# MinghanLi/STMask

Hardware: AMD Instinct MI355X
Metric: frames/sec at 360x640 R50-DCN-FPN (STMask hot path, fp32) (higher is better)
Workload: dtype f32

## Files before the change

### stmask_amd/csrc/head_sparse.hip

```cpp
#include <algorithm>

#include "stm_common.h"

namespace {

enum { CTL_RAW = 0,
       CTL_N = 1,
       CTL_FILL = 2,
       CTL_GATE_A = 3,
       CTL_GATE_B = 4,
       CTL_DENSE = 5,
       CTL_OVERFLOW = 6,
       CTL_GATE_POS = 7,
       CTL_INTS = 8 };

struct Levels {
    int n, B;
    int start[9], h[8], w[8];
};

__device__ __forceinline__ void decode_pixel(const Levels& L, int m, int& l, int& b, int& y, int& x)
{
    l = 0;
#pragma unroll
    for (int i = 1; i < 8; ++i)
        if (i < L.n && m >= L.start[i]) l = i;
    const int r = m - L.start[l], hw = L.h[l] * L.w[l];
    b = r / hw;
    const int p = r - b * hw;
    y = p / L.w[l];
    x = p - y * L.w[l];
}

struct CandArgs {
    const float* cls[4];
    int K, ld, n_cls, n_pixels, capacity;
    float thresh;
    int* list;
    int* ctl;
    int* flags;
    Levels L;
};

__global__ __launch_bounds__(256) void head_clear_kernel(int* ctl, int* flags, int n_pixels)
{
    const int i = blockIdx.x * 256 + threadIdx.x;
    if (i < n_pixels) flags[i] = 0;
    else if (i < n_pixels + CTL_INTS) ctl[i - n_pixels] = 0;
}

__device__ __forceinline__ void list_pixel(const CandArgs& a, int m)
{
    if (atomicCAS(a.flags + m, 0, 1) != 0) return;
    const int i = atomicAdd(a.ctl + CTL_RAW, 1);
    if (i < a.capacity) a.list[i] = m;
}

constexpr int CAND_PX = 64;

__global__ __launch_bounds__(256) void head_candidates_kernel(const CandArgs a, int vec)
{
    extern __shared__ float slab[];
    __shared__ unsigned kept_s[CAND_PX];
    const int stride = a.n_cls | 1;
    const int m0 = blockIdx.x * CAND_PX;
    const int rows = min(CAND_PX, a.n_pixels - m0);
    if (threadIdx.x < CAND_PX) kept_s[threadIdx.x] = 0u;
    for (int k = 0; k < a.K; ++k) {
        const float* src = a.cls[k] + (int64_t)m0 * a.ld;
        float* dst = slab + k * CAND_PX * stride;
        if (vec) {
            const int nv = (a.n_cls + 3) >> 2;
            for (int idx = threadIdx.x; idx < rows * nv; idx += 256) {
                const int r = idx / nv, v = idx - r * nv;
                const float4 q = *reinterpret_cast<const float4*>(src + (int64_t)r * a.ld + 4 * v);
                float* d = dst + r * stride + 4 * v;
                d[0] = q.x;
                if (4 * v + 1 < a.n_cls) d[1] = q.y;
// ... 4 lines not shown
            for (int idx = threadIdx.x; idx < rows * a.n_cls; idx += 256) {
                const int r = idx / a.n_cls, c = idx - r * a.n_cls;
                dst[r * stride + c] = src[(int64_t)r * a.ld + c];
            }
        }
    }
    __syncthreads();
    const int k = threadIdx.x / CAND_PX, r = threadIdx.x - k * CAND_PX;
    if (k < a.K && r < rows) {
        const float* row = slab + (k * CAND_PX + r) * stride;
        float mf = row[1];
        for (int c = 2; c < a.n_cls; ++c) mf = row[c] > mf ? row[c] : mf;
        const float mx = row[0] > mf ? row[0] : mf;
        float sum = 0.0f;
        for (int c = 0; c < a.n_cls; ++c) sum += expf(row[c] - mx);
        const float p = expf(mf - mx) / sum;
        if (p > a.thresh) atomicOr(&kept_s[r], 1u << k);
    }
    __syncthreads();
    if (threadIdx.x >= rows) return;
    const unsigned kept = kept_s[threadIdx.x];
    if (!kept) return;
    const int m = m0 + threadIdx.x;
    list_pixel(a, m);
    int l, b, y, x;
    decode_pixel(a.L, m, l, b, y, x);
    const int hw = a.L.h[l] * a.L.w[l], pix = y * a.L.w[l] + x;
    for (int kk = 0; kk < a.K; ++kk)
        if (kept >> kk & 1) list_pixel(a, a.L.start[l] + b * hw + (pix * a.K + kk) % hw);
}

__global__ void head_control_kernel(int* ctl, int capacity, int n_pixels, int px_a, int px_b)
{
    if (threadIdx.x || blockIdx.x) return;
    const int raw = ctl[CTL_RAW];
    const bool over = raw > capacity;
    const int n = over ? 0 : raw;
    const int fill = min(capacity, (n + 255) & ~255);
    ctl[CTL_N] = n;
    ctl[CTL_FILL] = fill;
    ctl[CTL_GATE_A] = fill * px_a;
    ctl[CTL_GATE_B] = fill * px_b;
    ctl[CTL_DENSE] = over ? n_pixels : 0;
    ctl[CTL_OVERFLOW] = over ? 1 : 0;
    ctl[CTL_GATE_POS] = n;
}

struct GatherArgs {
    const uint8_t* src;
    uint8_t* dst;
    int rows;
    int64_t src_np, dst_np;
    int S;
    const int* list;
    const int* ctl;
    Levels L;
};

__global__ __launch_bounds__(256) void head_patch_gather_kernel(const GatherArgs a)
{
    const int n = a.ctl[CTL_N], fill = a.ctl[CTL_FILL];
    const int SS = a.S * a.S, half = a.S >> 1;
    const int row_groups = (a.rows + 15) >> 4;
    const int64_t units = (int64_t)fill * SS * row_groups;
    const int lane = threadIdx.x & 63;
    const int sub_row = lane >> 2, chunk = lane & 3;
    for (int64_t u = (int64_t)blockIdx.x * 4 + (threadIdx.x >> 6); u < units; u += (int64_t)gridDim.x * 4) {
        const int64_t pp = u / row_groups;
// ... 26 lines not shown
        if (y - half >= 0 && y + half < L.h[l] && x - half >= 0 && x + half < L.w[l]) continue;
        const int work = SS * rows * 4;
        for (int t = threadIdx.x; t < work; t += 256) {
            const int chunk = t & 3, r = (t >> 2) % rows, q = (t >> 2) / rows;
            const int yy = y + q / S - half, xx = x + q % S - half;
            if ((unsigned)yy < (unsigned)L.h[l] && (unsigned)xx < (unsigned)L.w[l]) continue;
            *reinterpret_cast<uint4*>(planes + ((int64_t)r * np + (int64_t)i * SS + q) * 64 + chunk * 16) = make_uint4(0u, 0u, 0u, 0u);
        }
    }
}

struct AsmArgs {
    const float* cls[4];
    const float* small[4];
    const float* trk[4];
    float *conf, *loc, *mask, *track, *cen;
    int B, K, n_levels, n_cls, mask_dim, embed, gpad, cls_ld, small_ld, trk_ld, N;
    int lvl_start[9], lvl_hw[8], lvl_off[8];
    int vec4;
    int row_mul, row_add;
    const int* list;
    const int* ctl;
    int capacity;
};

__device__ __forceinline__ void assemble_rest(const AsmArgs& a, const float* sm, const float* tk, int64_t o, int64_t cen_idx, int sub)
{
    if (sub < 4) a.loc[o * 4 + sub] = sm[1 + sub];
    for (int c = sub; c < a.mask_dim; c += 16) a.mask[o * a.mask_dim + c] = sm[a.gpad + c];
    if (sub == 0) a.cen[cen_idx] = tanhf(sm[0]);
    float ss = 0.0f;
    if (a.vec4) {
        typedef float f4 __attribute__((ext_vector_type(4)));
        f4 v[4];
        const int nv = a.embed >> 2;
#pragma unroll
        for (int q = 0; q < 4; ++q) {
            const int c4 = sub + 16 * q;
            if (c4 < nv) {
                v[q] = *reinterpret_cast<const f4*>(tk + 4 * c4);
                ss = fmaf(v[q].x, v[q].x, ss); ss = fmaf(v[q].y, v[q].y, ss); ss = fmaf(v[q].z, v[q].z, ss); ss = fmaf(v[q].w, v[q].w, ss);
            }
        }
#pragma unroll
        for (int d = 8; d >= 1; d >>= 1) ss += __shfl_xor(ss, d);
        const float inv = 1.0f / fmaxf(sqrtf(ss), 1e-12f);
// ... 19 lines not shown
    const int64_t row = (int64_t)stm_xcd_block(((int64_t)a.B * a.N + 15) >> 4) * 16 + (threadIdx.x >> 4);
    if (row < 0 || row >= (int64_t)a.B * a.N) return;
    const int b = (int)(row / a.N), n = (int)(row - (int64_t)b * a.N);
    int l = 0;
#pragma unroll
    for (int i = 1; i < 8; ++i)
        if (i < a.n_levels && n >= a.lvl_off[i]) l = i;
    const int r = n - a.lvl_off[l];
    const int p = r / a.K, k = r - p * a.K;
    const int hw = a.lvl_hw[l];
    const int64_t src = (int64_t)a.lvl_start[l] + (int64_t)b * hw + p;
    const int64_t o = (int64_t)b * a.N + n;
    if (MODE == 0) {
        const float* cl = a.cls[k] + src * a.cls_ld;
        for (int c = sub; c < a.n_cls; c += 16) a.conf[o * a.n_cls + c] = cl[c];
    } else {
        assemble_rest(a, a.small[k] + src * a.small_ld, a.trk[k] + src * a.trk_ld, o, (int64_t)b * a.N + a.lvl_off[l] + (int64_t)k * hw + p, sub);
    }
}

__global__ __launch_bounds__(256) void head_assemble_listed_kernel(const AsmArgs a)
{
    const int n_pos = a.ctl[CTL_N];
    const int sub = threadIdx.x & 15;
    const int64_t units = (int64_t)n_pos * a.K;
    for (int64_t u = (int64_t)blockIdx.x * 16 + (threadIdx.x >> 4); u < units; u += (int64_t)gridDim.x * 16) {
        const int i = (int)(u / a.K), k = (int)(u - (int64_t)i * a.K);
        const int m = a.list[i];
        int l = 0;
#pragma unroll
        for (int j = 1; j < 8; ++j)
            if (j < a.n_levels && m >= a.lvl_start[j]) l = j;
        const int hw = a.lvl_hw[l];
        const int rr = m - a.lvl_start[l];
        const int b = rr / hw, p = rr - b * hw;
        const int nn = a.lvl_off[l] + p * a.K + k;
        const int64_t o = (int64_t)b * a.N + nn;
        const int64_t src = (int64_t)i * a.row_mul + a.row_add;
        assemble_rest(a, a.small[k] + src * a.small_ld, a.trk[k] + src * a.trk_ld, o, (int64_t)b * a.N + a.lvl_off[l] + (int64_t)k * hw + p, sub);
    }
}

bool fill_levels(Levels& L, int n_levels, int B, const int* lvl_start, const int* lvl_h, const int* lvl_w)
{
    if (n_levels <= 0 || n_levels > 8 || B <= 0 || !lvl_start || !lvl_h || !lvl_w || lvl_start[0] != 0) return false;
    L.n = n_levels; L.B = B;
    for (int l = 0; l < 8; ++l) {
        L.start[l] = l < n_levels ? lvl_start[l] : 0;
        L.h[l] = l < n_levels ? lvl_h[l] : 1;
        L.w[l] = l < n_levels ? lvl_w[l] : 1;
        if (l < n_levels && (lvl_h[l] <= 0 || lvl_w[l] <= 0 || lvl_start[l + 1] - lvl_start[l] != B * lvl_h[l] * lvl_w[l])) return false;
    }
    L.start[8] = 0;
    L.start[n_levels] = lvl_start[n_levels];
    return true;
}

}

extern "C" int stm_head_candidates_f32(const float* const* cls_logits, int K, int ld, int n_cls, float conf_thresh, int capacity,
                                       int patch_pixels_a, int patch_pixels_b, int n_levels, int B, const int* lvl_start, const int* lvl_h,
                                       const int* lvl_w, int* flags, int* list, int* ctl, stm_stream_t stream)
{
    const char* who = "stm_head_candidates_f32";
    STM_REQUIRE(cls_logits && list && ctl && flags, STM_ENULL, "%s: NULL argument", who);
    CandArgs a;
    STM_REQUIRE(fill_levels(a.L, n_levels, B, lvl_start, lvl_h, lvl_w), STM_EINVAL, "%s: bad level table", who);
    const int n_pixels = a.L.start[n_levels];
    STM_REQUIRE(K > 0 && K <= 4 && n_cls >= 2 && ld >= n_cls && n_pixels > 0 && capacity > 0 && patch_pixels_a > 0 && patch_pixels_b > 0 &&
                    (int64_t)capacity * std::max(patch_pixels_a, patch_pixels_b) < ((int64_t)1 << 30), STM_EINVAL, "%s: bad sizes", who);
    for (int k = 0; k < 4; ++k) {
        a.cls[k] = k < K ? cls_logits[k] : nullptr;
        STM_REQUIRE(k >= K || a.cls[k], STM_ENULL, "%s: input %d is NULL", who, k);
    }
    a.K = K; a.ld = ld; a.n_cls = n_cls; a.n_pixels = n_pixels; a.capacity = capacity; a.thresh = conf_thresh; a.list = list; a.ctl = ctl;
    a.flags = flags;
    hipLaunchKernelGGL(head_clear_kernel, dim3(stm_cdiv(n_pixels + CTL_INTS, 256)), dim3(256), 0, stm_hs(stream), ctl, flags, n_pixels);
    STM_CHECK_LAUNCH("head_clear_kernel");
    int vec = ld % 4 == 0 && 4 * ((n_cls + 3) / 4) <= ld;
    for (int k = 0; k < K; ++k) vec = vec && ((uintptr_t)a.cls[k] % 16) == 0;
    const size_t lds = (size_t)K * CAND_PX * (n_cls | 1) * sizeof(float);
    STM_REQUIRE(lds <= 48 * 1024, STM_EUNSUPPORTED, "%s: %d classes x %d shapes do not fit the staging buffer", who, n_cls, K);
    hipLaunchKernelGGL(head_candidates_kernel, dim3(stm_cdiv(n_pixels, CAND_PX)), dim3(256), lds, stm_hs(stream), a, vec);
    STM_CHECK_LAUNCH("head_candidates_kernel");
    hipLaunchKernelGGL(head_control_kernel, dim3(1), dim3(64), 0, stm_hs(stream), ctl, capacity, n_pixels, patch_pixels_a, patch_pixels_b);
    STM_CHECK_LAUNCH("head_control_kernel");
    return STM_OK;
}

extern "C" int stm_head_patch_gather(const void* src_planes, long long src_np, void* dst_planes, int side, int n_planes, int slabs,
                                     int capacity, int n_levels, int B, const int* lvl_start, const int* lvl_h, const int* lvl_w, const int* list,
                                     const int* ctl, stm_stream_t stream)
{
    const char* who = "stm_head_patch_gather";
    STM_REQUIRE(src_planes && dst_planes && list && ctl, STM_ENULL, "%s: NULL argument", who);
    STM_REQUIRE(n_planes > 0 && slabs > 0 && capacity > 0 && side > 0 && (side & 1) && src_np > 0 &&
                    (uintptr_t)src_planes % 16 == 0 && (uintptr_t)dst_planes % 16 == 0, STM_EINVAL, "%s: bad sizes or alignment", who);
    GatherArgs a;
    STM_REQUIRE(fill_levels(a.L, n_levels, B, lvl_start, lvl_h, lvl_w), STM_EINVAL, "%s: bad level table", who);
    STM_REQUIRE(src_np >= a.L.start[n_levels], STM_EINVAL, "%s: the source planes hold fewer pixels than the levels", who);
    a.src = static_cast<const uint8_t*>(src_planes); a.dst = static_cast<uint8_t*>(dst_planes);
    a.rows = n_planes * slabs; a.src_np = src_np; a.dst_np = (int64_t)capacity * side * side; a.S = side;
    a.list = list; a.ctl = ctl;
    const int64_t units = (int64_t)capacity * side * side * ((a.rows + 15) / 16);
    const unsigned grid = (unsigned)std::min<int64_t>((units + 3) / 4, 16384);
    hipLaunchKernelGGL(head_patch_gather_kernel, dim3(grid), dim3(256), 0, stm_hs(stream), a);
    STM_CHECK_LAUNCH("head_patch_gather_kernel");
    return STM_OK;
}
// ... 2 lines not shown
                                   const int* lvl_h, const int* lvl_w, const int* list, const int* ctl, stm_stream_t stream)
{
    const char* who = "stm_head_patch_mask";
    STM_REQUIRE(planes && list && ctl, STM_ENULL, "%s: NULL argument", who);
    STM_REQUIRE(n_planes > 0 && slabs > 0 && capacity > 0 && side > 0 && (side & 1) && (uintptr_t)planes % 16 == 0, STM_EINVAL, "%s: bad sizes or alignment", who);
    Levels L;
    STM_REQUIRE(fill_levels(L, n_levels, B, lvl_start, lvl_h, lvl_w), STM_EINVAL, "%s: bad level table", who);
    hipLaunchKernelGGL(head_patch_mask_kernel, dim3(std::min(capacity, 2048)), dim3(256), 0, stm_hs(stream), static_cast<uint8_t*>(planes), n_planes * slabs,
                       (int64_t)capacity * side * side, side, list, ctl, L);
    STM_CHECK_LAUNCH("head_patch_mask_kernel");
    return STM_OK;
}

extern "C" int stm_head_assemble_sparse_f32(const float* const* cls_logits, int cls_ld, const float* const* small, const float* const* trk,
                                            const float* const* small_dense, const float* const* trk_dense, const stm_head_layout* L,
                                            int row_mul, int row_add, const int* list, const int* ctl, int capacity, float* conf, float* loc,
                                            float* mask, float* track, float* centerness, stm_stream_t stream)
{
    const char* who = "stm_head_assemble_sparse_f32";
    STM_REQUIRE(cls_logits && small && trk && small_dense && trk_dense && L && list && ctl && conf && loc && mask && track && centerness, STM_ENULL,
                "%s: NULL argument", who);
    STM_REQUIRE(L->B > 0 && L->K > 0 && L->K <= 4 && L->n_levels > 0 && L->n_levels <= 8 && L->n_cls > 0 && cls_ld >= L->n_cls && L->mask_dim > 0 &&
                    L->mask_dim <= L->group_pad && L->embed_dim > 0 && L->group_pad >= 5 && L->small_ld >= L->group_pad + L->mask_dim &&
                    L->trk_ld >= L->embed_dim && capacity > 0 && row_mul > 0 && row_add >= 0 && row_add < row_mul, STM_EINVAL, "%s: bad layout", who);
    AsmArgs a;
    a.conf = conf; a.loc = loc; a.mask = mask; a.track = track; a.cen = centerness;
    a.B = L->B; a.K = L->K; a.n_levels = L->n_levels; a.n_cls = L->n_cls; a.mask_dim = L->mask_dim; a.embed = L->embed_dim;
    a.gpad = L->group_pad; a.cls_ld = cls_ld; a.small_ld = L->small_ld; a.trk_ld = L->trk_ld;
    a.row_mul = row_mul; a.row_add = row_add; a.list = list; a.ctl = ctl; a.capacity = capacity;
    int off = 0, start = 0;
    for (int l = 0; l < 8; ++l) {
        a.lvl_start[l] = l < L->n_levels ? L->lvl_start[l] : 0;
        a.lvl_hw[l] = l < L->n_levels ? L->lvl_hw[l] : 1;
        a.lvl_off[l] = off;
        if (l < L->n_levels) {
            STM_REQUIRE(L->lvl_hw[l] > 0 && L->lvl_start[l] == start, STM_EINVAL, "%s: level %d: bad pixel range", who, l);
            off += L->lvl_hw[l] * L->K;
            start += L->B * L->lvl_hw[l];
        }
    }
    a.lvl_start[8] = 0;
    a.N = off;
    const int64_t rows = (int64_t)a.B * a.N;
    const bool al = a.embed % 4 == 0 && a.embed <= 256 && a.trk_ld % 4 == 0 && ((uintptr_t)track % 16) == 0;
    auto set = [&](const float* const* sm, const float* const* tk) -> bool {
        a.vec4 = al;
        for (int k = 0; k < 4; ++k) {
            a.cls[k] = k < a.K ? cls_logits[k] : nullptr;
            a.small[k] = k < a.K ? sm[k] : nullptr;
            a.trk[k] = k < a.K ? tk[k] : nullptr;
            if (k < a.K && !(a.cls[k] && a.small[k] && a.trk[k])) return false;
// ... 15 lines not shown
```

### stmask_amd/ops.py

```python
import ctypes
import os

import torch

from . import _lib
from ._lib import DeformGeom, StmError, c_p, call


def _pair(v):
    return (v, v) if isinstance(v, int) else tuple(v)


def _dev(*ts):
    for t in ts:
        if t is not None and not t.is_cuda:
            raise StmError("stmask_amd ops need tensors on the MI355X (got a CPU tensor); there is no CPU fallback")


def _f32c(t):
    if t.dtype != torch.float32:
        raise StmError(f"expected float32, got {t.dtype}")
    return t if t.is_contiguous() else t.contiguous()


# ... 1579 lines not shown
    return out


def head_assemble(small, trk, B, sizes, n_cls, mask_dim, embed_dim, group_pad):
    _dev(*small, *trk)
    K = len(small)
    L, start = _head_layout(B, K, sizes, n_cls, mask_dim, embed_dim, group_pad, small[0].shape[-1], trk[0].shape[-1])
    N = K * sum(h * w for h, w in sizes)
    for t in list(small) + list(trk):
        if t.dtype != torch.float32 or not t.is_contiguous() or t.shape[0] != start:
            raise StmError("head_assemble: inputs must be contiguous fp32 matrices over all level pixels")
    dev = small[0].device
    conf = torch.empty(B, N, n_cls, device=dev)
    loc = torch.empty(B, N, 4, device=dev)
    mask = torch.empty(B, N, mask_dim, device=dev)
    track = torch.empty(B, N, embed_dim, device=dev)
    cen = torch.empty(B, N, 1, device=dev)
    call("stm_head_assemble_f32", _ptr4(small), _ptr4(trk), ctypes.byref(L), _p(conf), _p(loc), _p(mask), _p(track), _p(cen), _stream())
    return conf, loc, mask, track, cen


HEAD_CTL_RAW, HEAD_CTL_N, HEAD_CTL_FILL, HEAD_CTL_GATE_A, HEAD_CTL_GATE_B, HEAD_CTL_DENSE, HEAD_CTL_OVERFLOW, HEAD_CTL_INTS = 0, 1, 2, 3, 4, 5, 6, 8
HEAD_CTL_GATE_POS = 7


def conv_set_pixel_gate(ctl, index):
    _lib.lib().stm_conv_set_pixel_gate(ctl.data_ptr() + 4 * index)


def _level_arrays(B, sizes):
    n = len(sizes)
    st, hh, ww = (ctypes.c_int * 9)(), (ctypes.c_int * 8)(), (ctypes.c_int * 8)()
    start = 0
    for l, (h, w) in enumerate(sizes):
        st[l], hh[l], ww[l] = start, h, w
        start += B * h * w
    st[n] = start
    return n, st, hh, ww, start


def _head_layout(B, K, sizes, n_cls, mask_dim, embed_dim, group_pad, small_ld, trk_ld):
    L = _lib.HeadLayout()
    L.B, L.K, L.n_levels, L.n_cls, L.mask_dim, L.embed_dim, L.group_pad = B, K, len(sizes), n_cls, mask_dim, embed_dim, group_pad
    L.small_ld, L.trk_ld = small_ld, trk_ld
    start = 0
    for l, (h, w) in enumerate(sizes):
        L.lvl_start[l], L.lvl_hw[l] = start, h * w
        start += B * h * w
    return L, start


def _ptr4(ts):
    return (ctypes.c_void_p * 4)(*([t.data_ptr() for t in ts] + [0] * (4 - len(ts))))


def head_candidates(cls_logits, n_cls, conf_thresh, capacity, patch_pixels_a, patch_pixels_b, B, sizes):
    _dev(*cls_logits)
    n_px, ld = cls_logits[0].shape
    n, st, hh, ww, total = _level_arrays(B, sizes)
    for t in cls_logits:
        if t.dtype != torch.float32 or not t.is_contiguous() or tuple(t.shape) != (n_px, ld) or n_px != total:
            raise StmError("head_candidates: inputs must be contiguous fp32 matrices over all level pixels")
    dev = cls_logits[0].device
    lst = torch.empty(capacity, dtype=torch.int32, device=dev)
    ctl = torch.empty(HEAD_CTL_INTS, dtype=torch.int32, device=dev)
    flags = torch.empty(n_px, dtype=torch.int32, device=dev)
    call("stm_head_candidates_f32", _ptr4(cls_logits), len(cls_logits), ld, n_cls, conf_thresh, capacity, patch_pixels_a, patch_pixels_b, n, B, st,
         hh, ww, _p(flags), _p(lst), _p(ctl), _stream())
    return lst, ctl


def head_patch_gather(src, dst, side, capacity, B, sizes, lst, ctl):
    _dev(src, dst)
    if (src.dim() != 4 or dst.dim() != 4 or src.shape[3] != 32 or src.element_size() != 2 or dst.dtype != src.dtype or not src.is_contiguous()
            or not dst.is_contiguous() or tuple(dst.shape) != (src.shape[0], src.shape[1], capacity * side * side, 32)):
        raise StmError(f"head_patch_gather: planes {tuple(src.shape)} -> {tuple(dst.shape)} do not fit capacity {capacity}, side {side}")
    n, st, hh, ww, _ = _level_arrays(B, sizes)
    call("stm_head_patch_gather", _p(src), src.shape[2], _p(dst), side, src.shape[0], src.shape[1], capacity, n, B, st, hh, ww, _p(lst), _p(ctl),
         _stream())
    return dst


def head_patch_mask(planes, side, capacity, B, sizes, lst, ctl):
    _dev(planes)
    if planes.dim() != 4 or planes.shape[3] != 32 or planes.element_size() != 2 or not planes.is_contiguous() or planes.shape[2] != capacity * side * side:
        raise StmError(f"head_patch_mask: planes {tuple(planes.shape)} do not fit capacity {capacity}, side {side}")
    n, st, hh, ww, _ = _level_arrays(B, sizes)
    call("stm_head_patch_mask", _p(planes), side, planes.shape[0], planes.shape[1], capacity, n, B, st, hh, ww, _p(lst), _p(ctl), _stream())
    return planes


def head_assemble_sparse(cls_logits, small, trk, small_dense, trk_dense, B, sizes, n_cls, mask_dim, embed_dim, group_pad, row_mul, row_add, lst, ctl,
                         capacity):
    _dev(*cls_logits, *small, *trk, *small_dense, *trk_dense)
    K = len(cls_logits)
    L, start = _head_layout(B, K, sizes, n_cls, mask_dim, embed_dim, group_pad, small[0].shape[-1], trk[0].shape[-1])
    N = K * sum(h * w for h, w in sizes)
    for t in list(cls_logits) + list(small_dense) + list(trk_dense):
        if t.dtype != torch.float32 or not t.is_contiguous() or t.shape[0] != start:
            raise StmError("head_assemble_sparse: dense inputs must be contiguous fp32 matrices over all level pixels")
    for t, d in zip(list(small) + list(trk), list(small_dense) + list(trk_dense)):
        if t.dtype != torch.float32 or not t.is_contiguous() or t.shape[0] < capacity * row_mul or t.shape[-1] != d.shape[-1]:
            raise StmError("head_assemble_sparse: patch inputs must be contiguous fp32 matrices of capacity * row_mul rows, as wide as the dense ones")
    dev = cls_logits[0].device
    conf = torch.empty(B, N, n_cls, device=dev)
    loc = torch.empty(B, N, 4, device=dev)
    mask = torch.empty(B, N, mask_dim, device=dev)
    track = torch.empty(B, N, embed_dim, device=dev)
    cen = torch.empty(B, N, 1, device=dev)
    call("stm_head_assemble_sparse_f32", _ptr4(cls_logits), cls_logits[0].shape[-1], _ptr4(small), _ptr4(trk), _ptr4(small_dense), _ptr4(trk_dense),
         ctypes.byref(L), row_mul, row_add, _p(lst), _p(ctl), capacity, _p(conf), _p(loc), _p(mask), _p(track), _p(cen), _stream())
    return conf, loc, mask, track, cen


def deform_conv_fused_supported(C, O, kernel_size, has_mask, fmt, deformable_groups=1):
    kh, kw = _pair(kernel_size)
    g = DeformGeom(1, C, 8, 8, kh, kw, 1, 1, kh // 2, kw // 2, 1, 1, deformable_groups, 8, 8)
    return bool(_lib.lib().stm_deform_conv_fused_planar_supported(ctypes.byref(g), O, 1 if has_mask else 0, fmt))


def deform_conv_fused_tiles(B, Ho, Wo, O):
    wide = O % 256 == 0 and os.environ.get("STM_DCN_FUSED_WIDE", "1") != "0"
    tp, bn = (64, 256) if wide else (128, 128)
    best, bt, bper = -1.0, 1, 1 << 30
    for tw in range(4, tp + 1):
        th = tp // tw
        if th < 1:
            break
        thc, twc = min(th, Ho), min(tw, Wo)
        tiles = -(-Ho // thc) * -(-Wo // twc)
        eff = Ho * Wo / (tiles * float(tp))
        per = thc + twc
        if eff > best + 1e-9 or (eff > best - 1e-9 and per < bper):
            best, bt, bper = eff, tiles, per
# ... 61 lines not shown
```

### stmask_amd/planar.py

```python
import ctypes
import functools
import os
from typing import Any, NamedTuple, Optional

import torch
import torch.nn.functional as F

from . import _lib, ops
from ._lib import StmError, call
from .ops import _pair


FMT = 0
BACKBONE_FMT = None

TILE64_MAX_SLABS = 8
FCB_PLANAR = True
STEM_PLANAR = True
C3DS_FUSED = True
STEM_FUSED = True
CONV_KXR = True
TN_BORDER = True
TN_POOL = True
CONV_CHAIN = True
# ... 64 lines not shown
                self._packed[tile_n] = ops.conv_pack_weights(self.weight, self.planes, tile_n)
        return self._packed[tile_n]

    def kxr_rule_pixels(self):
        return 20000 if self.groups > 1 else 30000

    def pick_tile(self, M):
        if self.tile_n is not None:
            return self.tile_n
        cg = self.O // self.groups
        if self.groups > 1 and cg % 128 != 0:
            return 64
        if cg <= 64 or (cg % 128 != 0 and cg % 128 <= 64 and cg < 256):
            return 64
        tiles128 = -(-M // 128) * -(-self.O // 128)
        slabs = self.C * self.kh * self.kw // 32
        if tiles128 < 400 and not (192 <= tiles128 <= 256 and slabs >= 64):
            return 64
        if slabs <= TILE64_MAX_SLABS:
            return 64
        return 128

    def __call__(self, xp, shape, out="planes", x_off=0, out_planes=None, out_f32=None, out_off=0, residual=None, x_ch_off=0,
                 out_ch_off=0, x2=None, window=None, gate=None, kxr=None, splitk=True):
        NP, dt = ops.plane_layout(self.fmt)
        if xp.dtype != dt or xp.dim() != 4 or xp.shape[0] < NP or xp.shape[3] != 32 or not xp.is_contiguous():
            raise StmError(f"PlanarConv: expected contiguous {dt} planes [{NP}, S, N, 32], got {xp.dtype} {tuple(xp.shape)}")
        S, N = xp.shape[1], xp.shape[2]
        g = _lib.ConvGeom()
        g.C, g.Cout, g.kh, g.kw, g.sh, g.sw, g.ph, g.pw = self.C, self.O, self.kh, self.kw, self.sh, self.sw, self.ph, self.pw
        g.planes, g.groups = self.planes, self.groups
        if self.group_cout:
            for i, c in enumerate(self.group_cout):
                g.group_cout[i] = c
        c_first = self.C - (x2[0].shape[1] * 32 if x2 is not None else 0)
        if S * 32 < x_ch_off + self.groups * c_first or x_ch_off % 32:
            raise StmError(f"PlanarConv: input has {S * 32} channels, layer reads {self.groups} x {c_first} from channel {x_ch_off}")
        if shape[0] == "levels":
            _, B, sizes = shape
            g.n_levels = len(sizes)
            start = 0
            for l, (h, w) in enumerate(sizes):
                g.lvl_start[l], g.lvl_h[l], g.lvl_w[l] = start, h, w
                start += B * h * w
            g.lvl_start[len(sizes)] = start
            M = start
            if x_off or N != start:
# ... 16 lines not shown
        one_px = window is not None and tuple(window[:4]) == (0, 0, 1, 1) and tuple(window[6:]) == (1, 1)
        use_kxr = (self.kxr and residual is None and (one_px if window is not None else (shape[0] == "levels" or (Ho, Wo) == (H, W)))
                   and (kxr if kxr is not None else M >= (self.kxr_min_pixels if self.kxr_min_pixels is not None else self.kxr_rule_pixels())))
        g.tile_n = 0 if use_kxr else self.pick_tile(M)
        dev = xp.device
        NPo, dto = ops.plane_layout(self.out_fmt)
        if window is not None and ((out in ("planes", "both") and out_planes is None) or (out in ("f32", "both") and out_f32 is None)):
            raise StmError("PlanarConv: a window launch writes into caller-provided full-size outputs")
        if out in ("planes", "both") and out_planes is None:
            out_planes, out_off_p = torch.empty(NPo, -(-self.O // 32), M, 32, device=dev, dtype=dto), 0
        else:
            out_off_p = out_off
        if out in ("f32", "both") and out_f32 is None:
            out_f32, out_off_f = torch.empty(M, self.O, device=dev, dtype=torch.float32), 0
        else:
            out_off_f = out_off
        if out == "planes":
            out_f32 = None
        if out == "f32":
            out_planes = None
        p_pl = p_f32 = 0
        if out_planes is not None:
            g.out_np, g.out_plane_stride = out_planes.shape[2], out_planes.shape[1] * out_planes.shape[2] * 32
            p_pl = out_planes.data_ptr() + out_off_p * 64
        if out_f32 is not None:
            g.out_ld = out_f32.shape[-1]
            p_f32 = out_f32.data_ptr() + (out_off_f * g.out_ld + out_ch_off) * 4
        r32 = rpl = 0
        if residual is not None:
            if residual.dtype == dt:
                if residual.shape[0] < NP:
                    raise StmError(f"PlanarConv: residual has {residual.shape[0]} plane(s), format {self.fmt} reads {NP}")
                g.res_np, g.res_plane_stride = residual.shape[2], residual.shape[1] * residual.shape[2] * 32
                rpl = residual.data_ptr()
            else:
                g.res_ld = residual.shape[-1]
                r32 = residual.data_ptr()
        started = _timing_start()
        x_ptr = xp.data_ptr() + ((x_ch_off // 32) * N + x_off) * 64
        if use_kxr:
            g.fmt = self.fmt
            if "kxr" not in self._packed:
                ops.planar_range_flag()
                self._packed["kxr"] = ops.conv_pack_weights_kxr(self.weight, g, wscale=self.wscale)
            packed, g.out_scale = self._packed["kxr"]
            if gate is not None:
                ops.conv_set_pixel_gate(*gate)
# ... 29 lines not shown
                                            dilation, has_mask=has_mask, relu=self.relu, fmt=self.fmt, out_fmt=self.out_fmt, out=out, out_off=out_off)

    def _algo_bytes(self, M, shape, NP, NPo, dt, out_f32, out_planes, residual):
        in_px = M if shape[0] == "levels" else shape[1] * shape[2] * shape[3]
        nbytes = in_px * self.groups * self.C * 2 * NP + self.weight.numel() * 2 * NP
        if out_planes is not None:
            nbytes += M * self.O * 2 * NPo
        if out_f32 is not None:
            nbytes += M * self.O * 4
        if residual is not None:
            nbytes += M * self.O * (2 * NP if residual.dtype == dt else 4)
        return nbytes


def _nhwc(t):
    return t.permute(0, 2, 3, 1).contiguous()


def _split(t_nhwc, fmt=None):
    return ops.split_planes(t_nhwc, FMT if fmt is None else fmt)


@functools.lru_cache(maxsize=None)
def head_center_default():
    return os.environ.get("STM_HEAD_CENTER", "1") != "0"


class HeadOutputs(NamedTuple):
    small: PlanarConv
    trk: PlanarConv
    fa: Optional[Any] = None
    fconv: Optional[PlanarConv] = None
    adconv: Optional[PlanarConv] = None
    adfused: Optional[PlanarConv] = None


class _Levels(NamedTuple):
    B: int
    sizes: tuple
    starts: tuple
    ntot: int
    dev: torch.device

    @property
    def lv(self):
        return ("levels", self.B, self.sizes)
# ... 4 lines not shown

    def __init__(self, net):
        cfg = net.cfg
        self.net = net
        self.fmt = FMT
        fpn = net.fpn
        self.n_lat = len(fpn.lat_layers)
        self.fpn_pred = [PlanarConv(m.weight, m.bias, m.stride, m.padding, relu=True) for m in fpn.pred_layers]
        self.fpn_down = [PlanarConv(m.weight, m.bias, m.stride, m.padding, relu=False) for m in fpn.downsample_layers]
        self.fpn_lat = [PlanarConv(m.weight, m.bias, 1, 0, relu=False) for m in fpn.lat_layers]
        self.proto = []
        mods = [m for m in net.proto_net.children() if not isinstance(m, (torch.nn.ReLU, torch.nn.Identity))]
        for m in mods:
            if isinstance(m, torch.nn.Conv2d):
                self.proto.append(PlanarConv(m.weight, m.bias, m.stride, m.padding, relu=True))
            else:
                self.proto.append(m)
        self.cor_idx = net.correlation_selected_layer if cfg.temporal_fusion_module else None
        self.timer = None
        head = net.prediction_layers[0]
        self.head_planar = not (cfg.use_dcn_track or cfg.use_dcn_mask) and cfg.share_prediction_module
        self.fcb = bool(cfg.use_dcn_class)
        self.sparse = None
        self._sparse_layers = None
        self.sparse_ctl = self.sparse_list = None
        self._side = None
        if not self.head_planar:
            return
        convs = lambda seq: [m for m in seq.children() if isinstance(m, torch.nn.Conv2d)]
        up = convs(head.upfeature)
        assert len(up) == 1
        self.up = PlanarConv(up[0].weight, up[0].bias, 1, up[0].padding, relu=True)
        towers = [convs(head.conf_extra), convs(head.bbox_extra), convs(head.mask_extra), convs(head.track_extra)]
        assert all(len(t) == 2 for t in towers), "extra_layers (2,2,2,2) is the only head layout on the hot path"
        w1 = torch.cat([t[0].weight for t in towers], 0)
        b1 = torch.cat([t[0].bias for t in towers], 0)
        self.tower1 = PlanarConv(w1, b1, 1, towers[0][0].padding, relu=True)
        w2 = torch.cat([t[1].weight for t in towers], 0)
        b2 = torch.cat([t[1].bias for t in towers], 0)
        self.tower2 = PlanarConv(w2, b2, 1, towers[0][1].padding, relu=True, groups=4)
        self.dims = (head.num_priors * head.num_classes, head.num_priors * 4, head.num_priors * head.mask_dim,
                     head.num_priors * head.embed_dim)
        self.finals = [self._head_outputs(head, k) for k in range(len(cfg.head_layer_params))]
        self.head = head

    def _head_outputs(self, head, k):
        P = self.GROUP_PAD
# ... 41 lines not shown
        s0, s1, s2 = self.SPARSE_SIDES
        per_frame = max(1, 2 * sum(h * w for h, w in sizes) // (s1 * s1 + s2 * s2))
        return -(-per_frame * B // 256) * 256

    def _build_sparse(self):
        if self._sparse_layers is not None:
            return self._sparse_layers
        P = self.GROUP_PAD
        cw = self.tower2.O // 4

        def cut(layer, rows, **kw):
            c = PlanarConv(layer.weight[rows], layer.bias[rows], 1, (layer.ph, layer.pw), relu=layer.relu, fmt=layer.fmt, **kw)
            c.wscale = ops._pow2_wscale(layer.weight) if layer.fmt >= 1 else None
            return c

        t1c, t1r = cut(self.tower1, slice(0, cw)), cut(self.tower1, slice(cw, 4 * cw))
        t2c, t2r = cut(self.tower2, slice(0, cw)), cut(self.tower2, slice(cw, 4 * cw), groups=3)
        cls, small = [], []
        for sm in (f.small for f in self.finals):
            gc = sm.group_cout
            cls.append(cut(sm, slice(0, P), tile_n=64, group_cout=gc[:1], algo_frac=gc[0] / float(P)))
            small.append(cut(sm, slice(P, 3 * P), groups=2, tile_n=64, group_cout=gc[1:], algo_frac=sum(gc[1:]) / (2.0 * P)))
        self._sparse_layers = (t1c, t1r, t2c, t2r, cls, small)
        return self._sparse_layers

    def _sparse_head(self, up, g, toc):
        head, (B, sizes, _, ntot, dev) = self.head, g
        thresh, cap = self.sparse[:2]
        center = self.sparse[2] if len(self.sparse) > 2 else head_center_default()
        if cap is None:
            cap = self.sparse_capacity(B, sizes)
        t1c, t1r, t2c, t2r, cls_l, small_l = self._build_sparse()
        trk_l = [f.trk for f in self.finals]
        lv = g.lv
        cw, P = self.tower2.O // 4, self.GROUP_PAD
        S0, S1, S2 = self.SPARSE_SIDES
        NP, pdt = ops.plane_layout(self.fmt)
        kx = ntot >= self.finals[0].small.kxr_rule_pixels()
        x = t1c(up, lv, out="planes", splitk=False)
        x = t2c(x, lv, out="planes", splitk=False)
        cls = [c(x, lv, out="f32", splitk=False, kxr=kx) for c in cls_l]
        toc("head_towers")
        lst, ctl = ops.head_candidates(cls, head.num_classes, thresh, cap, S1 * S1, S2 * S2, B, sizes)
        patch = ops.head_patch_gather(up, torch.empty(NP, cw // 32, cap * S0 * S0, 32, device=dev, dtype=pdt), S0, cap, B, sizes, lst, ctl)
        x1 = torch.empty(NP, 3 * cw // 32, cap * S1 * S1, 32, device=dev, dtype=pdt)
        t1r(patch, ("img", cap, S0, S0), out="planes", out_planes=x1, window=(0, 0, S1, S1, 0, 0, S1, S1), gate=(ctl, ops.HEAD_CTL_GATE_A))
        ops.head_patch_mask(x1, S1, cap, B, sizes, lst, ctl)
        gb = (ctl, ops.HEAD_CTL_GATE_B)
        xq = torch.empty(NP, 3 * cw // 32, cap * S2 * S2, 32, device=dev, dtype=pdt)
        t2r(x1, ("img", cap, S1, S1), out="planes", out_planes=xq, window=(0, 0, S2, S2, 0, 0, S2, S2), gate=gb)
        ops.head_patch_mask(xq, S2, cap, B, sizes, lst, ctl)
        if center:
            c2, gp = S2 // 2, (ctl, ops.HEAD_CTL_GATE_POS)
            qi = ("img", cap, S2, S2)

            def centre(c, **kw):
                return c(xq, qi, out="f32", out_f32=torch.empty(cap, c.O, device=dev), window=(0, 0, 1, 1, c.ph - c2, c.pw - c2, 1, 1), gate=gp, **kw)

            small = [centre(c, kxr=kx) for c in small_l]
            trk = [centre(c, x_ch_off=2 * cw, kxr=False) for c in trk_l]
            rows = (1, 0)
        else:
            ql = ("levels", cap, [(S2, S2)])
            small = [c(xq, ql, out="f32", gate=gb, kxr=kx) for c in small_l]
            trk = [c(xq, ql, out="f32", x_ch_off=2 * cw, gate=gb) for c in trk_l]
            rows = (S2 * S2, (S2 * S2) // 2)
        gd = (ctl, ops.HEAD_CTL_DENSE)
        x = t1r(up, lv, out="planes", gate=gd)
        x = t2r(x, lv, out="planes", gate=gd)
        small_d = [c(x, lv, out="f32", gate=gd, kxr=kx) for c in small_l]
        trk_d = [c(x, lv, out="f32", x_ch_off=2 * cw, gate=gd) for c in trk_l]
        toc("head_finals")
        out = ops.head_assemble_sparse(cls, small, trk, small_d, trk_d, B, sizes, head.num_classes, head.mask_dim, head.embed_dim, P,
                                       rows[0], rows[1], lst, ctl, cap)
        self.sparse_ctl, self.sparse_list = ctl, lst
        return out

    def run(self, bb_outs, planes=None):
        toc = self.timer.toc if self.timer is not None else (lambda name: None)
        toc("backbone")
        lat, latp, B, sizes = self._fpn_laterals(bb_outs, planes)
        toc("fpn_lateral")
        for d in self.fpn_down:
            h, w = sizes[-1]
            sizes.append(ops.conv_out_hw(h, w, d.kh, d.kw, d.sh, d.sw, d.ph, d.pw, 1, 1))
        starts = [0]
        for h, w in sizes:
            starts.append(starts[-1] + B * h * w)
        g = _Levels(B, tuple(sizes), tuple(starts), starts[-1], (latp[0] if latp[0] is not None else lat[0]).device)
        side = self._side_stream(g.dev, B)
        feat, fpn_outs = self._fpn_levels(g, lat, latp, side)
        toc("fpn_pred_down")
        proto_side = side is not None and TRUNK_BRANCHES >= 1 and self.head_planar
        if proto_side:
            main = torch.cuda.current_stream()
            side.wait_stream(main)
            with torch.cuda.stream(side), ops.workspace_branch("proto"):
# ... 572 lines not shown
```

### stmask_amd/trunk.py

```python
import os
import sys
import time

import torch

from . import ops, planar

_SIDE_STREAMS = {}


def concurrent_side_streams(dev, n=2):
    dev = torch.device(dev)
    main = torch.cuda.current_stream(dev)
    key = (dev.index, main.cuda_stream)
    have = _SIDE_STREAMS.get(key, [])
    if len(have) >= n:
        return have[:n]
    cands = [torch.cuda.Stream(device=dev) for _ in range(16)]
    chosen = list(have)
    spin = getattr(torch.cuda, "_sleep", None)
    if spin is not None and not torch.cuda.is_current_stream_capturing():
        cycles = 1_000_000

        def run(streams):
# ... 26 lines not shown


class TrunkRunner:

    PREFETCH_DEPTH = int(os.environ.get("STM_PREFETCH_DEPTH", "3"))
    N_GRAPH_SLOTS = 2 * PREFETCH_DEPTH + 2
    LARGE_BATCH = 8

    def __init__(self, net, n_clips, timer):
        self.net, self.cfg, self.B = net, net.cfg, n_clips
        self.tf = bool(self.cfg.temporal_fusion_module)
        self.timer = timer
        self._pending = []
        self._sides = []
        self._side_next = 0
        self.prefetch_early = True
        self.use_graph = False
        self._graph_sparse = None
        self._sparse_now = None
        self._graph_planes = None
        self._reset_graphs()
        self.sparse_head = os.environ.get("STM_SPARSE_HEAD", "1") != "0"
        self.head_center = planar.head_center_default()
        self.sparse_min_clips = int(os.environ.get("STM_SPARSE_MIN_CLIPS", "4"))
        self.sparse_capacity = None

    def _reset_graphs(self):
        self._graphs = []
        self._graph_ws = []
        self._graph_next = 0
        self._graph_warm = 0
        self.graph_active = False

    @property
    def prefetch_depth(self):
        return self.PREFETCH_DEPTH if self.B <= self.LARGE_BATCH else min(self.PREFETCH_DEPTH, 2)

    @property
    def n_graph_slots(self):
        return 2 * self.prefetch_depth + 2

    def _sparse_setting(self, pg):
        if not (self.sparse_head and self.B >= self.sparse_min_clips and self.tf and pg is not None and pg.sparse_supported()):
            return None
        if not getattr(self.net.Detect_TF, "use_cross_class_nms", True):
            return None
        return (float(self.cfg.eval_conf_thresh), self.sparse_capacity, self.head_center)

    def _trunk(self, frames):
        pg = getattr(self.net, "_planar", None)
        if pg is None:
            return self._trunk_run(frames)
        self._sparse_now = self._sparse_setting(pg)
        before, pg.sparse = pg.sparse, self._sparse_now
        try:
            return self._trunk_run(frames)
        finally:
            pg.sparse = before

    def _trunk_run(self, frames):
        net = self.net
        if not (self.use_graph and getattr(net, "_planar", None) is not None and not self.timer.on and ops._conv_timing is None
                and ops._im2col_timing is None):
            return net.forward_single(frames)
        planes = getattr(net, "_planar_planes", None)
        if self._graphs and (self._graph_planes != planes or self._graph_sparse != self._sparse_now):
            self._pending = []
            torch.cuda.synchronize()
            self._reset_graphs()
        if self._graph_warm < 2:
# ... 81 lines not shown
```

Baseline: 1798.

## Split sparse head candidates into owned and partner pixels, skipping mask/track work for partners

Candidate pixels are now flagged as either owning a confident anchor or only being a partner location. A new list kernel orders owned pixels first and keeps separate control counts. The mask and track tower branches and the track finals are then gated to owned pixels only, while the box branch still runs for all listed pixels. This cuts convolution work in the sparse head, at the cost of an extra list kernel, extra atomics, and more conv launches because the towers are split.

```diff
diff --git a/stmask_amd/csrc/head_sparse.hip b/stmask_amd/csrc/head_sparse.hip
--- a/stmask_amd/csrc/head_sparse.hip
+++ b/stmask_amd/csrc/head_sparse.hip
@@ -1,4 +1,5 @@
 #include <algorithm>
+#include <climits>
 
 #include "stm_common.h"
 
@@ -12,7 +13,9 @@
        CTL_DENSE = 5,
        CTL_OVERFLOW = 6,
        CTL_GATE_POS = 7,
-       CTL_INTS = 8 };
+       CTL_INTS = 8,
+       CTL_OWN = 8 };
+enum { FLAG_OWN = 1, FLAG_PARTNER = 2 };
 
 struct Levels {
     int n, B;
@@ -39,14 +42,15 @@
     int* list;
     int* ctl;
     int* flags;
+    int split;
     Levels L;
 };
 
-__global__ __launch_bounds__(256) void head_clear_kernel(int* ctl, int* flags, int n_pixels)
+__global__ __launch_bounds__(256) void head_clear_kernel(int* ctl, int* flags, int n_flags, int n_ctl)
 {
     const int i = blockIdx.x * 256 + threadIdx.x;
-    if (i < n_pixels) flags[i] = 0;
-    else if (i < n_pixels + CTL_INTS) ctl[i - n_pixels] = 0;
+    if (i < n_flags) flags[i] = 0;
+    else if (i < n_flags + n_ctl) ctl[i - n_flags] = 0;
 }
 
 __device__ __forceinline__ void list_pixel(const CandArgs& a, int m)
@@ -54,6 +58,13 @@
     if (atomicCAS(a.flags + m, 0, 1) != 0) return;
     const int i = atomicAdd(a.ctl + CTL_RAW, 1);
     if (i < a.capacity) a.list[i] = m;
+}
+
+__device__ __forceinline__ void flag_pixel(const CandArgs& a, int m, int bit)
+{
+    const int old = atomicOr(a.flags + m, bit);
+    if (old == 0) atomicAdd(a.ctl + CTL_RAW, 1);
+    if (bit == FLAG_OWN && !(old & FLAG_OWN)) atomicAdd(a.ctl + CTL_OWN + CTL_RAW, 1);
 }
 
 constexpr int CAND_PX = 64;
@@ -104,28 +115,52 @@
     const unsigned kept = kept_s[threadIdx.x];
     if (!kept) return;
     const int m = m0 + threadIdx.x;
-    list_pixel(a, m);
+    if (a.split) flag_pixel(a, m, FLAG_OWN);
+    else list_pixel(a, m);
     int l, b, y, x;
     decode_pixel(a.L, m, l, b, y, x);
     const int hw = a.L.h[l] * a.L.w[l], pix = y * a.L.w[l] + x;
     for (int kk = 0; kk < a.K; ++kk)
-        if (kept >> kk & 1) list_pixel(a, a.L.start[l] + b * hw + (pix * a.K + kk) % hw);
-}
-
-__global__ void head_control_kernel(int* ctl, int capacity, int n_pixels, int px_a, int px_b)
-{
-    if (threadIdx.x || blockIdx.x) return;
-    const int raw = ctl[CTL_RAW];
-    const bool over = raw > capacity;
-    const int n = over ? 0 : raw;
+        if (kept >> kk & 1) {
+            const int pm = a.L.start[l] + b * hw + (pix * a.K + kk) % hw;
+            if (a.split) flag_pixel(a, pm, FLAG_PARTNER);
+            else list_pixel(a, pm);
+        }
+}
+
+__global__ void head_control_kernel(int* ctl, int capacity, int n_pixels, int px_a, int px_b, int blocks)
+{
+    if (blockIdx.x || (int)threadIdx.x >= blocks) return;
+    const bool over = ctl[CTL_RAW] > capacity;
+    int* c = ctl + threadIdx.x * CTL_OWN;
+    const int n = over ? 0 : c[CTL_RAW];
     const int fill = min(capacity, (n + 255) & ~255);
-    ctl[CTL_N] = n;
-    ctl[CTL_FILL] = fill;
-    ctl[CTL_GATE_A] = fill * px_a;
-    ctl[CTL_GATE_B] = fill * px_b;
-    ctl[CTL_DENSE] = over ? n_pixels : 0;
-    ctl[CTL_OVERFLOW] = over ? 1 : 0;
-    ctl[CTL_GATE_POS] = n;
+    c[CTL_N] = n;
+    c[CTL_FILL] = fill;
+    c[CTL_GATE_A] = fill * px_a;
+    c[CTL_GATE_B] = fill * px_b;
+    c[CTL_DENSE] = over ? n_pixels : 0;
+    c[CTL_OVERFLOW] = over ? 1 : 0;
+    c[CTL_GATE_POS] = n;
+}
+
+__global__ __launch_bounds__(256) void head_list_kernel(const int* flags, int* cursors, int n_pixels, int capacity, int* list, const int* ctl)
+{
+    __shared__ int cnt_s[2], base_s[2];
+    if (threadIdx.x < 2) cnt_s[threadIdx.x] = 0;
+    __syncthreads();
+    const int n = ctl[CTL_N], n_own = ctl[CTL_OWN + CTL_N];
+    const int m = blockIdx.x * 256 + threadIdx.x;
+    const int f = m < n_pixels && n > 0 ? flags[m] : 0;
+    const int cls = f & FLAG_OWN ? 0 : (f ? 1 : -1);
+    int rank = 0;
+    if (cls >= 0) rank = atomicAdd(&cnt_s[cls], 1);
+    __syncthreads();
+    if (threadIdx.x < 2) base_s[threadIdx.x] = cnt_s[threadIdx.x] ? atomicAdd(cursors + threadIdx.x, cnt_s[threadIdx.x]) : 0;
+    __syncthreads();
+    if (cls < 0) return;
+    const int i = (cls ? n_own : 0) + base_s[cls] + rank;
+    if (i < n && i < capacity) list[i] = m;
 }
 
 struct GatherArgs {
@@ -198,6 +233,7 @@
     const int* list;
     const int* ctl;
     int capacity;
+    int split;
 };
 
 __device__ __forceinline__ void assemble_rest(const AsmArgs& a, const float* sm, const float* tk, int64_t o, int64_t cen_idx, int sub)
@@ -263,6 +299,7 @@
 __global__ __launch_bounds__(256) void head_assemble_listed_kernel(const AsmArgs a)
 {
     const int n_pos = a.ctl[CTL_N];
+    const int n_own = a.split ? a.ctl[CTL_OWN + CTL_N] : n_pos;
     const int sub = threadIdx.x & 15;
     const int64_t units = (int64_t)n_pos * a.K;
     for (int64_t u = (int64_t)blockIdx.x * 16 + (threadIdx.x >> 4); u < units; u += (int64_t)gridDim.x * 16) {
@@ -278,7 +315,14 @@
         const int nn = a.lvl_off[l] + p * a.K + k;
         const int64_t o = (int64_t)b * a.N + nn;
         const int64_t src = (int64_t)i * a.row_mul + a.row_add;
-        assemble_rest(a, a.small[k] + src * a.small_ld, a.trk[k] + src * a.trk_ld, o, (int64_t)b * a.N + a.lvl_off[l] + (int64_t)k * hw + p, sub);
+        const int64_t cen_idx = (int64_t)b * a.N + a.lvl_off[l] + (int64_t)k * hw + p;
+        if (i >= n_own) {
+            const float* sm = a.small[k] + src * a.small_ld;
+            if (sub < 4) a.loc[o * 4 + sub] = sm[1 + sub];
+            if (sub == 0) a.cen[cen_idx] = tanhf(sm[0]);
+            continue;
+        }
+        assemble_rest(a, a.small[k] + src * a.small_ld, a.trk[k] + src * a.trk_ld, o, cen_idx, sub);
     }
 }
 
@@ -308,6 +352,9 @@
     CandArgs a;
     STM_REQUIRE(fill_levels(a.L, n_levels, B, lvl_start, lvl_h, lvl_w), STM_EINVAL, "%s: bad level table", who);
     const int n_pixels = a.L.start[n_levels];
+    const int split = capacity < 0;
+    STM_REQUIRE(capacity != INT_MIN, STM_EINVAL, "%s: bad sizes", who);
+    if (split) capacity = -capacity;
     STM_REQUIRE(K > 0 && K <= 4 && n_cls >= 2 && ld >= n_cls && n_pixels > 0 && capacity > 0 && patch_pixels_a > 0 && patch_pixels_b > 0 &&
                     (int64_t)capacity * std::max(patch_pixels_a, patch_pixels_b) < ((int64_t)1 << 30), STM_EINVAL, "%s: bad sizes", who);
     for (int k = 0; k < 4; ++k) {
@@ -315,8 +362,9 @@
         STM_REQUIRE(k >= K || a.cls[k], STM_ENULL, "%s: input %d is NULL", who, k);
     }
     a.K = K; a.ld = ld; a.n_cls = n_cls; a.n_pixels = n_pixels; a.capacity = capacity; a.thresh = conf_thresh; a.list = list; a.ctl = ctl;
-    a.flags = flags;
-    hipLaunchKernelGGL(head_clear_kernel, dim3(stm_cdiv(n_pixels + CTL_INTS, 256)), dim3(256), 0, stm_hs(stream), ctl, flags, n_pixels);
+    a.flags = flags; a.split = split;
+    const int n_flags = n_pixels + (split ? 2 : 0), n_ctl = split ? 2 * CTL_INTS : CTL_INTS;
+    hipLaunchKernelGGL(head_clear_kernel, dim3(stm_cdiv(n_flags + n_ctl, 256)), dim3(256), 0, stm_hs(stream), ctl, flags, n_flags, n_ctl);
     STM_CHECK_LAUNCH("head_clear_kernel");
     int vec = ld % 4 == 0 && 4 * ((n_cls + 3) / 4) <= ld;
     for (int k = 0; k < K; ++k) vec = vec && ((uintptr_t)a.cls[k] % 16) == 0;
@@ -324,8 +372,13 @@
     STM_REQUIRE(lds <= 48 * 1024, STM_EUNSUPPORTED, "%s: %d classes x %d shapes do not fit the staging buffer", who, n_cls, K);
     hipLaunchKernelGGL(head_candidates_kernel, dim3(stm_cdiv(n_pixels, CAND_PX)), dim3(256), lds, stm_hs(stream), a, vec);
     STM_CHECK_LAUNCH("head_candidates_kernel");
-    hipLaunchKernelGGL(head_control_kernel, dim3(1), dim3(64), 0, stm_hs(stream), ctl, capacity, n_pixels, patch_pixels_a, patch_pixels_b);
+    hipLaunchKernelGGL(head_control_kernel, dim3(1), dim3(64), 0, stm_hs(stream), ctl, capacity, n_pixels, patch_pixels_a, patch_pixels_b,
+                       split ? 2 : 1);
     STM_CHECK_LAUNCH("head_control_kernel");
+    if (split) {
+        hipLaunchKernelGGL(head_list_kernel, dim3(stm_cdiv(n_pixels, 256)), dim3(256), 0, stm_hs(stream), flags, flags + n_pixels, n_pixels, capacity, list, ctl);
+        STM_CHECK_LAUNCH("head_list_kernel");
+    }
     return STM_OK;
 }
 
@@ -374,11 +427,13 @@
                 "%s: NULL argument", who);
     STM_REQUIRE(L->B > 0 && L->K > 0 && L->K <= 4 && L->n_levels > 0 && L->n_levels <= 8 && L->n_cls > 0 && cls_ld >= L->n_cls && L->mask_dim > 0 &&
                     L->mask_dim <= L->group_pad && L->embed_dim > 0 && L->group_pad >= 5 && L->small_ld >= L->group_pad + L->mask_dim &&
-                    L->trk_ld >= L->embed_dim && capacity > 0 && row_mul > 0 && row_add >= 0 && row_add < row_mul, STM_EINVAL, "%s: bad layout", who);
+                    L->trk_ld >= L->embed_dim && capacity != 0 && capacity != INT_MIN && row_mul > 0 && row_add >= 0 && row_add < row_mul, STM_EINVAL, "%s: bad layout", who);
     AsmArgs a;
     a.conf = conf; a.loc = loc; a.mask = mask; a.track = track; a.cen = centerness;
     a.B = L->B; a.K = L->K; a.n_levels = L->n_levels; a.n_cls = L->n_cls; a.mask_dim = L->mask_dim; a.embed = L->embed_dim;
     a.gpad = L->group_pad; a.cls_ld = cls_ld; a.small_ld = L->small_ld; a.trk_ld = L->trk_ld;
+    a.split = capacity < 0;
+    if (a.split) capacity = -capacity;
     a.row_mul = row_mul; a.row_add = row_add; a.list = list; a.ctl = ctl; a.capacity = capacity;
     int off = 0, start = 0;
     for (int l = 0; l < 8; ++l) {
diff --git a/stmask_amd/ops.py b/stmask_amd/ops.py
--- a/stmask_amd/ops.py
+++ b/stmask_amd/ops.py
@@ -1625,6 +1625,7 @@
 
 HEAD_CTL_RAW, HEAD_CTL_N, HEAD_CTL_FILL, HEAD_CTL_GATE_A, HEAD_CTL_GATE_B, HEAD_CTL_DENSE, HEAD_CTL_OVERFLOW, HEAD_CTL_INTS = 0, 1, 2, 3, 4, 5, 6, 8
 HEAD_CTL_GATE_POS = 7
+HEAD_CTL_OWN = 8
 
 
 def conv_set_pixel_gate(ctl, index):
@@ -1657,7 +1658,7 @@
     return (ctypes.c_void_p * 4)(*([t.data_ptr() for t in ts] + [0] * (4 - len(ts))))
 
 
-def head_candidates(cls_logits, n_cls, conf_thresh, capacity, patch_pixels_a, patch_pixels_b, B, sizes):
+def head_candidates(cls_logits, n_cls, conf_thresh, capacity, patch_pixels_a, patch_pixels_b, B, sizes, split=False):
     _dev(*cls_logits)
     n_px, ld = cls_logits[0].shape
     n, st, hh, ww, total = _level_arrays(B, sizes)
@@ -1666,9 +1667,9 @@
             raise StmError("head_candidates: inputs must be contiguous fp32 matrices over all level pixels")
     dev = cls_logits[0].device
     lst = torch.empty(capacity, dtype=torch.int32, device=dev)
-    ctl = torch.empty(HEAD_CTL_INTS, dtype=torch.int32, device=dev)
-    flags = torch.empty(n_px, dtype=torch.int32, device=dev)
-    call("stm_head_candidates_f32", _ptr4(cls_logits), len(cls_logits), ld, n_cls, conf_thresh, capacity, patch_pixels_a, patch_pixels_b, n, B, st,
+    ctl = torch.empty(HEAD_CTL_INTS * (2 if split else 1), dtype=torch.int32, device=dev)
+    flags = torch.empty(n_px + (2 if split else 0), dtype=torch.int32, device=dev)
+    call("stm_head_candidates_f32", _ptr4(cls_logits), len(cls_logits), ld, n_cls, conf_thresh, -capacity if split else capacity, patch_pixels_a, patch_pixels_b, n, B, st,
          hh, ww, _p(flags), _p(lst), _p(ctl), _stream())
     return lst, ctl
 
@@ -1694,7 +1695,9 @@
 
 
 def head_assemble_sparse(cls_logits, small, trk, small_dense, trk_dense, B, sizes, n_cls, mask_dim, embed_dim, group_pad, row_mul, row_add, lst, ctl,
-                         capacity):
+                         capacity, split=False):
+    if ctl.numel() < HEAD_CTL_INTS * (2 if split else 1):
+        raise StmError("head_assemble_sparse: the split form reads a control block of 16 ints")
     _dev(*cls_logits, *small, *trk, *small_dense, *trk_dense)
     K = len(cls_logits)
     L, start = _head_layout(B, K, sizes, n_cls, mask_dim, embed_dim, group_pad, small[0].shape[-1], trk[0].shape[-1])
@@ -1712,7 +1715,7 @@
     track = torch.empty(B, N, embed_dim, device=dev)
     cen = torch.empty(B, N, 1, device=dev)
     call("stm_head_assemble_sparse_f32", _ptr4(cls_logits), cls_logits[0].shape[-1], _ptr4(small), _ptr4(trk), _ptr4(small_dense), _ptr4(trk_dense),
-         ctypes.byref(L), row_mul, row_add, _p(lst), _p(ctl), capacity, _p(conf), _p(loc), _p(mask), _p(track), _p(cen), _stream())
+         ctypes.byref(L), row_mul, row_add, _p(lst), _p(ctl), -capacity if split else capacity, _p(conf), _p(loc), _p(mask), _p(track), _p(cen), _stream())
     return conf, loc, mask, track, cen
 
 
diff --git a/stmask_amd/planar.py b/stmask_amd/planar.py
--- a/stmask_amd/planar.py
+++ b/stmask_amd/planar.py
@@ -110,7 +110,7 @@
         return 128
 
     def __call__(self, xp, shape, out="planes", x_off=0, out_planes=None, out_f32=None, out_off=0, residual=None, x_ch_off=0,
-                 out_ch_off=0, x2=None, window=None, gate=None, kxr=None, splitk=True):
+                 out_ch_off=0, x2=None, window=None, gate=None, kxr=None, splitk=True, out_slab_off=0):
         NP, dt = ops.plane_layout(self.fmt)
         if xp.dtype != dt or xp.dim() != 4 or xp.shape[0] < NP or xp.shape[3] != 32 or not xp.is_contiguous():
             raise StmError(f"PlanarConv: expected contiguous {dt} planes [{NP}, S, N, 32], got {xp.dtype} {tuple(xp.shape)}")
@@ -173,7 +173,9 @@
         p_pl = p_f32 = 0
         if out_planes is not None:
             g.out_np, g.out_plane_stride = out_planes.shape[2], out_planes.shape[1] * out_planes.shape[2] * 32
-            p_pl = out_planes.data_ptr() + out_off_p * 64
+            if out_slab_off < 0 or out_slab_off + -(-self.O // 32) > out_planes.shape[1]:
+                raise StmError(f"PlanarConv: {self.O} output channels from slab {out_slab_off} run past the {out_planes.shape[1]} slabs of out_planes")
+            p_pl = out_planes.data_ptr() + (out_slab_off * g.out_np + out_off_p) * 64
         if out_f32 is not None:
             g.out_ld = out_f32.shape[-1]
             p_f32 = out_f32.data_ptr() + (out_off_f * g.out_ld + out_ch_off) * 4
@@ -249,6 +251,11 @@
 
 
 @functools.lru_cache(maxsize=None)
+def head_split_default():
+    return os.environ.get("STM_HEAD_SPLIT", "1") != "0"
+
+
+@functools.lru_cache(maxsize=None)
 def head_center_default():
     return os.environ.get("STM_HEAD_CENTER", "1") != "0"
 
@@ -299,7 +306,7 @@
         self.head_planar = not (cfg.use_dcn_track or cfg.use_dcn_mask) and cfg.share_prediction_module
         self.fcb = bool(cfg.use_dcn_class)
         self.sparse = None
-        self._sparse_layers = None
+        self._sparse_layers = self._split_layers = None
         self.sparse_ctl = self.sparse_list = None
         self._side = None
         if not self.head_planar:
@@ -387,12 +394,16 @@
             cls.append(cut(sm, slice(0, P), tile_n=64, group_cout=gc[:1], algo_frac=gc[0] / float(P)))
             small.append(cut(sm, slice(P, 3 * P), groups=2, tile_n=64, group_cout=gc[1:], algo_frac=sum(gc[1:]) / (2.0 * P)))
         self._sparse_layers = (t1c, t1r, t2c, t2r, cls, small)
+        self._split_layers = (cut(self.tower1, slice(cw, 2 * cw)), cut(self.tower1, slice(2 * cw, 4 * cw)),
+                              cut(self.tower2, slice(cw, 2 * cw)), cut(self.tower2, slice(2 * cw, 4 * cw), groups=2))
         return self._sparse_layers
 
     def _sparse_head(self, up, g, toc):
         head, (B, sizes, _, ntot, dev) = self.head, g
         thresh, cap = self.sparse[:2]
         center = self.sparse[2] if len(self.sparse) > 2 else head_center_default()
+        split = len(self.sparse) > 3 and bool(self.sparse[3])
+        own = ops.HEAD_CTL_OWN if split else 0
         if cap is None:
             cap = self.sparse_capacity(B, sizes)
         t1c, t1r, t2c, t2r, cls_l, small_l = self._build_sparse()
@@ -406,29 +417,39 @@
         x = t2c(x, lv, out="planes", splitk=False)
         cls = [c(x, lv, out="f32", splitk=False, kxr=kx) for c in cls_l]
         toc("head_towers")
-        lst, ctl = ops.head_candidates(cls, head.num_classes, thresh, cap, S1 * S1, S2 * S2, B, sizes)
+        lst, ctl = ops.head_candidates(cls, head.num_classes, thresh, cap, S1 * S1, S2 * S2, B, sizes, split=split)
         patch = ops.head_patch_gather(up, torch.empty(NP, cw // 32, cap * S0 * S0, 32, device=dev, dtype=pdt), S0, cap, B, sizes, lst, ctl)
         x1 = torch.empty(NP, 3 * cw // 32, cap * S1 * S1, 32, device=dev, dtype=pdt)
-        t1r(patch, ("img", cap, S0, S0), out="planes", out_planes=x1, window=(0, 0, S1, S1, 0, 0, S1, S1), gate=(ctl, ops.HEAD_CTL_GATE_A))
-        ops.head_patch_mask(x1, S1, cap, B, sizes, lst, ctl)
+        xq = torch.empty(NP, 3 * cw // 32, cap * S2 * S2, 32, device=dev, dtype=pdt)
         gb = (ctl, ops.HEAD_CTL_GATE_B)
-        xq = torch.empty(NP, 3 * cw // 32, cap * S2 * S2, 32, device=dev, dtype=pdt)
-        t2r(x1, ("img", cap, S1, S1), out="planes", out_planes=xq, window=(0, 0, S2, S2, 0, 0, S2, S2), gate=gb)
+        w1, w2 = (0, 0, S1, S1, 0, 0, S1, S1), (0, 0, S2, S2, 0, 0, S2, S2)
+        if split:
+            t1b, t1m, t2b, t2m = self._split_layers
+            t1b(patch, ("img", cap, S0, S0), out="planes", out_planes=x1, window=w1, gate=(ctl, ops.HEAD_CTL_GATE_A))
+            t1m(patch, ("img", cap, S0, S0), out="planes", out_planes=x1, out_slab_off=cw // 32, window=w1, gate=(ctl, own + ops.HEAD_CTL_GATE_A))
+            ops.head_patch_mask(x1, S1, cap, B, sizes, lst, ctl)
+            t2b(x1, ("img", cap, S1, S1), out="planes", out_planes=xq, window=w2, gate=gb)
+            t2m(x1, ("img", cap, S1, S1), out="planes", out_planes=xq, x_ch_off=cw, out_slab_off=cw // 32, window=w2, gate=(ctl, own + ops.HEAD_CTL_GATE_B))
+        else:
+            t1r(patch, ("img", cap, S0, S0), out="planes", out_planes=x1, window=w1, gate=(ctl, ops.HEAD_CTL_GATE_A))
+            ops.head_patch_mask(x1, S1, cap, B, sizes, lst, ctl)
+            t2r(x1, ("img", cap, S1, S1), out="planes", out_planes=xq, window=w2, gate=gb)
         ops.head_patch_mask(xq, S2, cap, B, sizes, lst, ctl)
         if center:
-            c2, gp = S2 // 2, (ctl, ops.HEAD_CTL_GATE_POS)
+            c2 = S2 // 2
             qi = ("img", cap, S2, S2)
 
-            def centre(c, **kw):
-                return c(xq, qi, out="f32", out_f32=torch.empty(cap, c.O, device=dev), window=(0, 0, 1, 1, c.ph - c2, c.pw - c2, 1, 1), gate=gp, **kw)
-
-            small = [centre(c, kxr=kx) for c in small_l]
-            trk = [centre(c, x_ch_off=2 * cw, kxr=False) for c in trk_l]
+            def centre(c, blk, **kw):
+                return c(xq, qi, out="f32", out_f32=torch.empty(cap, c.O, device=dev), window=(0, 0, 1, 1, c.ph - c2, c.pw - c2, 1, 1),
+                         gate=(ctl, blk + ops.HEAD_CTL_GATE_POS), **kw)
+
+            small = [centre(c, 0, kxr=kx) for c in small_l]
+            trk = [centre(c, own, x_ch_off=2 * cw, kxr=False) for c in trk_l]
             rows = (1, 0)
         else:
             ql = ("levels", cap, [(S2, S2)])
             small = [c(xq, ql, out="f32", gate=gb, kxr=kx) for c in small_l]
-            trk = [c(xq, ql, out="f32", x_ch_off=2 * cw, gate=gb) for c in trk_l]
+            trk = [c(xq, ql, out="f32", x_ch_off=2 * cw, gate=(ctl, own + ops.HEAD_CTL_GATE_B)) for c in trk_l]
             rows = (S2 * S2, (S2 * S2) // 2)
         gd = (ctl, ops.HEAD_CTL_DENSE)
         x = t1r(up, lv, out="planes", gate=gd)
@@ -437,7 +458,7 @@
         trk_d = [c(x, lv, out="f32", x_ch_off=2 * cw, gate=gd) for c in trk_l]
         toc("head_finals")
         out = ops.head_assemble_sparse(cls, small, trk, small_d, trk_d, B, sizes, head.num_classes, head.mask_dim, head.embed_dim, P,
-                                       rows[0], rows[1], lst, ctl, cap)
+                                       rows[0], rows[1], lst, ctl, cap, split=split)
         self.sparse_ctl, self.sparse_list = ctl, lst
         return out
 
diff --git a/stmask_amd/trunk.py b/stmask_amd/trunk.py
--- a/stmask_amd/trunk.py
+++ b/stmask_amd/trunk.py
@@ -72,6 +72,7 @@
         self._reset_graphs()
         self.sparse_head = os.environ.get("STM_SPARSE_HEAD", "1") != "0"
         self.head_center = planar.head_center_default()
+        self.head_split = planar.head_split_default()
         self.sparse_min_clips = int(os.environ.get("STM_SPARSE_MIN_CLIPS", "4"))
         self.sparse_capacity = None
 
@@ -95,7 +96,7 @@
             return None
         if not getattr(self.net.Detect_TF, "use_cross_class_nms", True):
             return None
-        return (float(self.cfg.eval_conf_thresh), self.sparse_capacity, self.head_center)
+        return (float(self.cfg.eval_conf_thresh), self.sparse_capacity, self.head_center, self.head_split)
 
     def _trunk(self, frames):
         pg = getattr(self.net, "_planar", None)
```

Result: faster. 1838, median of 6 (+2.2%).
